# SparkJiao/llama-pipeline-parallel

Hardware: AMD Instinct MI355X
Metric: tokens/sec (whole node), LLaMA-65B PP=8 seq4096 at 1/2/4/8 MI355X (higher is better)
Workload: dtype bf16; 1 GPU; model=llama-65b, measured_model=llama-65b-shaped 10-layer slice (10/80 layers), global_batch=64, seq_len=4096, parallelism=pp1, num_layers=10, micro_batch_size=4, grad_accum_steps=16

## Files before the change

### lpp_amd/ops/csrc/attention_api.cpp

```cpp
#include <string>
#include <vector>

#include "attention.h"

namespace lpp {

static int g_order_mode = [] {
  const char* e = getenv("LPP_ATTN_ORDER");
  return (e && e[0] == '0') ? 0 : 1;
}();

int attn_order_mode() { return g_order_mode; }

void attn_check_qkv(const at::Tensor& q, const at::Tensor& k, const at::Tensor& v,
                    const char* who) {
  TORCH_CHECK(q.is_cuda() && q.scalar_type() == at::kBFloat16, who, ": bf16 only");
  TORCH_CHECK(q.dim() == 4 && q.size(3) == ATTN_D, who, ": [B,S,H,128] required");
  TORCH_CHECK(q.is_contiguous() && k.is_contiguous() && v.is_contiguous());
  TORCH_CHECK(q.size(2) % k.size(2) == 0);
}

static void attn_check_bwd(const at::Tensor& dO, const at::Tensor& q, const at::Tensor& k,
                           const at::Tensor& v, const at::Tensor& o,
                           const at::Tensor& lse2, const char* who) {
// ... 24 lines not shown
  auto dv = at::empty_like(v);
  const int mode = lpp::attn_order_mode();
  lpp::launch_attn_bwd_dq(dO, q, k, v, lse2, delta, dq, mode ? lpp::ATTN_MODE1_DQ : 0, 0);
  lpp::launch_attn_bwd_dkdv(dO, q, k, v, lse2, delta, dk, dv,
                            mode ? lpp::ATTN_MODE1_DKDV : 0, 0);
  return {dq, dk, dv};
}

void attention_set_block_order(int64_t mode) {
  TORCH_CHECK(mode == 0 || mode == 1, "attention_set_block_order: mode 0 or 1");
  lpp::g_order_mode = (int)mode;
}

int64_t attention_get_block_order() { return lpp::g_order_mode; }

at::Tensor attention_block_order(int64_t kind, int64_t nblk, int64_t nheads, int64_t G,
                                 int64_t mode) {
  TORCH_CHECK(kind == 0 || kind == 1, "attention_block_order: kind 0 (fwd/dQ) or 1 (dK/dV)");
  TORCH_CHECK(mode == 0 || mode == 1, "attention_block_order: mode 0 or 1");
  TORCH_CHECK(nblk >= 1 && nheads >= 1 && nblk * nheads < (int64_t)1 << 30 && G >= 1);
  G = std::min(G, nheads);
  const int n = (int)(nblk * nheads);
  auto out = at::empty({n, 2}, at::TensorOptions().dtype(at::kInt));
  int* p = out.data_ptr<int>();
  for (int L = 0; L < n; ++L) {
    const lpp::AttnBlock ob =
        lpp::attn_block_order(L, (int)nblk, (int)nheads, (int)G, (int)kind, (int)mode);
    p[2 * L] = ob.blk;
    p[2 * L + 1] = ob.head;
  }
  return out;
}

std::vector<double> attention_time_kernel(std::string kernel, at::Tensor dO, at::Tensor q,
                                          at::Tensor k, at::Tensor v, at::Tensor o,
                                          at::Tensor lse2, int64_t mode, int64_t G,
                                          int64_t warmup, int64_t reps) {
  lpp::attn_check_bwd(dO, q, k, v, o, lse2, "attention_time_kernel");
  TORCH_CHECK(mode == 0 || mode == 1, "attention_time_kernel: mode 0 or 1");
  TORCH_CHECK(kernel == "fwd" || kernel == "dq" || kernel == "dkdv",
              "attention_time_kernel: kernel is fwd, dq or dkdv");
  const int B = q.size(0), S = q.size(1), H = q.size(2);
  auto delta = at::empty({B, H, S}, q.options().dtype(at::kFloat));
  lpp::launch_attn_bwd_delta(dO, o, delta);
  auto o2 = at::empty_like(q), dq = at::empty_like(q);
  auto lse_out = at::empty_like(lse2);
  auto dk = at::empty_like(k), dv = at::empty_like(v);
  auto launch = [&] {
    if (kernel == "fwd") lpp::launch_attn_fwd(q, k, v, o2, lse_out, (int)mode, (int)G);
    else if (kernel == "dq")
      lpp::launch_attn_bwd_dq(dO, q, k, v, lse2, delta, dq, (int)mode, (int)G);
    else lpp::launch_attn_bwd_dkdv(dO, q, k, v, lse2, delta, dk, dv, (int)mode, (int)G);
  };
  auto stream = lpp::current_stream();
  hipEvent_t e0, e1;
  LPP_CHECK_HIP(hipEventCreate(&e0));
  LPP_CHECK_HIP(hipEventCreate(&e1));
  for (int64_t i = 0; i < warmup; ++i) launch();
  std::vector<double> ms;
  for (int64_t i = 0; i < reps; ++i) {
    LPP_CHECK_HIP(hipEventRecord(e0, stream));
    launch();
    LPP_CHECK_HIP(hipEventRecord(e1, stream));
    LPP_CHECK_HIP(hipEventSynchronize(e1));
    float t = 0.f;
    LPP_CHECK_HIP(hipEventElapsedTime(&t, e0, e1));
// ... 7 lines not shown
```

### lpp_amd/ops/csrc/attention_bwd.hip

```cpp
#include "attention.h"

namespace lpp {

__global__ __launch_bounds__(256) void attn_bwd_delta_kernel(
    const short* __restrict__ dO, const short* __restrict__ O,
    float* __restrict__ delta, int64_t rows, int S, int H) {
  const int lg = threadIdx.x & 15;
  const int grp = (blockIdx.x * 256 + (int)threadIdx.x) >> 4;
  const int64_t stride = ((int64_t)gridDim.x * 256) >> 4;
  for (int64_t r = grp; r < rows; r += stride) {
    const bf16x8 d8 = *reinterpret_cast<const bf16x8*>(&dO[r * ATTN_D + lg * 8]);
    const bf16x8 o8 = *reinterpret_cast<const bf16x8*>(&O[r * ATTN_D + lg * 8]);
    float acc = 0.f;
#pragma unroll
    for (int j = 0; j < 8; ++j) acc += bf16_to_f32(d8[j]) * bf16_to_f32(o8[j]);
#pragma unroll
    for (int m = 1; m < 16; m <<= 1) acc += __shfl_xor(acc, m);
    if (lg == 0) {
      const int h = (int)(r % H);
      const int64_t bs = r / H;
      const int s = (int)(bs % S);
      const int64_t b = bs / S;
      delta[(b * H + h) * S + s] = acc;
    }
  }
}

constexpr int DQ_QW = 32, DQ_QB = 256, DQ_KVB = ATTN_TILE_ROWS;
enum { DQ_K, DQ_V, DQ_KT, DQ_IMAGES };
constexpr int DQ_LDS_BYTES = attn_lds_bytes(DQ_IMAGES);

__global__ __launch_bounds__(512, 2) void attn_bwd_dq_kernel(
    const short* __restrict__ Q, const short* __restrict__ K,
    const short* __restrict__ V, const short* __restrict__ dO,
    const float* __restrict__ LSE2, const float* __restrict__ Delta,
    short* __restrict__ dQ,
    int B, int S, int H, int HKV, float c, float scale,
    int order_mode, int order_G) {
  extern __shared__ __attribute__((aligned(16))) char smem[];
  auto k_lds = [&](int buf) -> char* { return attn_img(smem, DQ_K, buf); };
  auto v_lds = [&](int buf) -> char* { return attn_img(smem, DQ_V, buf); };
  auto kt_lds = [&](int buf) -> char* { return attn_img(smem, DQ_KT, buf); };

  const int tid = threadIdx.x;
  const int wid = __builtin_amdgcn_readfirstlane(tid >> 6);
  const int lane = tid & 63;
  const int lq = lane & 31;
  const int hi2 = lane >> 5;

  const AttnBlock ob = attn_block_order(blockIdx.x, (S + DQ_QB - 1) / DQ_QB, B * H,
                                        order_G, ATTN_ORDER_FWD_DQ, order_mode);
  const int qblk = ob.blk;
  const int b = ob.head / H;
  const int h = ob.head % H;
  const int hkv = h / (H / HKV);
  const int64_t sHD = (int64_t)H * ATTN_D;
  const int64_t sHkvD = (int64_t)HKV * ATTN_D;
  const int64_t q_base = (((int64_t)b * S) * H + h) * ATTN_D;
  const int64_t kv_base = (((int64_t)b * S) * HKV + hkv) * ATTN_D;
  const int64_t ld_base = ((int64_t)b * H + h) * S;

  const int qw0 = qblk * DQ_QB + wid * DQ_QW;
  const int qrow = qw0 + lq;

  bf16x8 qf[8], dof[8];
  {
    const int64_t rb = q_base + (int64_t)min(qrow, S - 1) * sHD;
#pragma unroll
    for (int dc = 0; dc < 8; ++dc) {
      qf[dc] = *reinterpret_cast<const bf16x8*>(&Q[rb + dc * 16 + hi2 * 8]);
      dof[dc] = *reinterpret_cast<const bf16x8*>(&dO[rb + dc * 16 + hi2 * 8]);
    }
  }
  const float Lq = LSE2[ld_base + min(qrow, S - 1)];
  const float Dq = Delta[ld_base + min(qrow, S - 1)];

  const int st_r = lane >> 4;
  const int st_c = 8 * (lane & 15);
  const int kv_end = min(S, (qblk + 1) * DQ_QB);

  auto ld_tile = [&](int kv0, int pass, bf16x8& kreg, bf16x8& vreg) {
    const int row = min(kv0 + stage_row(wid, pass, st_r), S - 1);
    const int64_t rb = kv_base + (int64_t)row * sHkvD + st_c;
    kreg = *reinterpret_cast<const bf16x8*>(&K[rb]);
    vreg = *reinterpret_cast<const bf16x8*>(&V[rb]);
  };
  auto write_tile = [&](int buf, int pass, bf16x8 kreg, bf16x8 vreg) {
    const int r = stage_row(wid, pass, st_r);
    stage_normal(k_lds(buf), r, st_c, kreg);
    stage_normal(v_lds(buf), r, st_c, vreg);
    stage_transposed(kt_lds(buf), r, st_c, st_r, kreg);
  };

  f32x16 dq_acc[4];
#pragma unroll
  for (int dt = 0; dt < 4; ++dt)
#pragma unroll
    for (int r = 0; r < 16; ++r) dq_acc[dt][r] = 0.f;

  bf16x8 kreg0, kreg1, vreg0, vreg1;
  ld_tile(0, 0, kreg0, vreg0);
  ld_tile(0, 1, kreg1, vreg1);
  write_tile(0, 0, kreg0, vreg0);
  write_tile(0, 1, kreg1, vreg1);
  if (DQ_KVB < kv_end) {
    ld_tile(DQ_KVB, 0, kreg0, vreg0);
    ld_tile(DQ_KVB, 1, kreg1, vreg1);
  }
  __syncthreads();
  for (int kv0 = 0, cur = 0; kv0 < kv_end; kv0 += DQ_KVB, cur ^= 1) {
    if (kv0 + DQ_KVB < kv_end) {
      write_tile(cur ^ 1, 0, kreg0, vreg0);
      write_tile(cur ^ 1, 1, kreg1, vreg1);
      if (kv0 + 2 * DQ_KVB < kv_end) {
        ld_tile(kv0 + 2 * DQ_KVB, 0, kreg0, vreg0);
        ld_tile(kv0 + 2 * DQ_KVB, 1, kreg1, vreg1);
      }
    }
    if (kv0 < qw0 + DQ_QW) {
      const bool need_mask = (kv0 + DQ_KVB > qw0) || (kv0 + DQ_KVB > S);
#pragma unroll
      for (int t2 = 0; t2 < 2; ++t2) {
        f32x16 st, dpt;
#pragma unroll
        for (int r = 0; r < 16; ++r) { st[r] = 0.f; dpt[r] = 0.f; }
        __builtin_amdgcn_s_setprio(1);
#pragma unroll
        for (int dc = 0; dc < 8; ++dc) {
          const bf16x8 ak = *reinterpret_cast<const bf16x8*>(
              k_lds(cur) + rswz(t2 * 32 + lq, dc * 16 + hi2 * 8));
          const bf16x8 av = *reinterpret_cast<const bf16x8*>(
              v_lds(cur) + rswz(t2 * 32 + lq, dc * 16 + hi2 * 8));
          st = __builtin_amdgcn_mfma_f32_32x32x16_bf16(ak, qf[dc], st, 0, 0, 0);
          dpt = __builtin_amdgcn_mfma_f32_32x32x16_bf16(av, dof[dc], dpt, 0, 0, 0);
        }
        __builtin_amdgcn_s_setprio(0);

        float ds[16];
        if (need_mask) {
#pragma unroll
          for (int r = 0; r < 16; ++r) {
            const int kv = kv0 + t2 * 32 + crow32(r, hi2);
            const bool ok = (kv <= qrow) && (kv < S);
            const float e = exp2f(fmaf(st[r], c, -Lq));
            ds[r] = (ok ? e : 0.f) * (dpt[r] - Dq);
          }
        } else {
#pragma unroll
          for (int r = 0; r < 16; ++r)
            ds[r] = exp2f(fmaf(st[r], c, -Lq)) * (dpt[r] - Dq);
        }

        bf16x8 dsa[2];
        pack_pair(ds, dsa);

        __builtin_amdgcn_s_setprio(1);
#pragma unroll
        for (int dt = 0; dt < 4; ++dt) {
          const int d = dt * 32 + lq;
#pragma unroll
          for (int ks = 0; ks < 2; ++ks) {
            const bf16x8 bk = *reinterpret_cast<const bf16x8*>(
                kt_lds(cur) + tswz(d, (2 * t2 + ks) * 16 + hi2 * 8));
            dq_acc[dt] = __builtin_amdgcn_mfma_f32_32x32x16_bf16(dsa[ks], bk, dq_acc[dt], 0, 0, 0);
          }
        }
        __builtin_amdgcn_s_setprio(0);
      }
    }
    __syncthreads();
  }

#pragma unroll
  for (int r = 0; r < 16; ++r) {
    const int row = qw0 + crow32(r, hi2);
    if (row >= S) continue;
    const int64_t rb = q_base + (int64_t)row * sHD;
#pragma unroll
    for (int dt = 0; dt < 4; ++dt)
      dQ[rb + dt * 32 + lq] = f32_to_bf16(dq_acc[dt][r] * scale);
  }
}

constexpr int KV_KW = 16, KV_WG = 128, KV_QT = ATTN_TILE_ROWS;
enum { KV_Q, KV_DO, KV_QTR, KV_DOTR, KV_IMAGES };
constexpr int KV_LD_OFF = attn_lds_bytes(KV_IMAGES);
constexpr int KV_D_OFF = KV_LD_OFF + 2 * KV_QT * (int)sizeof(float);
constexpr int KV_LDS_BYTES = KV_D_OFF + 2 * KV_QT * (int)sizeof(float);

__global__ __launch_bounds__(512, 2) void attn_bwd_dkdv_kernel(
    const short* __restrict__ Q, const short* __restrict__ K,
    const short* __restrict__ V, const short* __restrict__ dO,
    const float* __restrict__ LSE2, const float* __restrict__ Delta,
    short* __restrict__ dK, short* __restrict__ dV,
    int B, int S, int H, int HKV, float c, float scale,
    int order_mode, int order_G) {
  extern __shared__ __attribute__((aligned(16))) char smem[];
  auto q_lds = [&](int buf) -> char* { return attn_img(smem, KV_Q, buf); };
  auto do_lds = [&](int buf) -> char* { return attn_img(smem, KV_DO, buf); };
  auto qt_lds = [&](int buf) -> char* { return attn_img(smem, KV_QTR, buf); };
  auto dot_lds = [&](int buf) -> char* { return attn_img(smem, KV_DOTR, buf); };
  auto l_buf = [&](int buf) -> float* {
    return reinterpret_cast<float*>(smem + KV_LD_OFF) + buf * KV_QT; };
  auto d_buf = [&](int buf) -> float* {
    return reinterpret_cast<float*>(smem + KV_D_OFF) + buf * KV_QT; };

  const int tid = threadIdx.x;
  const int wid = __builtin_amdgcn_readfirstlane(tid >> 6);
  const int lane = tid & 63;
  const int l16 = lane & 15;
  const int hi4 = (lane >> 4) & 3;

  const AttnBlock ob = attn_block_order(blockIdx.x, (S + KV_WG - 1) / KV_WG, B * HKV,
                                        order_G, ATTN_ORDER_DKDV, order_mode);
  const int kvblk = ob.blk;
  const int b = ob.head / HKV;
  const int hkv = ob.head % HKV;
  const int G = H / HKV;
  const int64_t sHD = (int64_t)H * ATTN_D;
  const int64_t sHkvD = (int64_t)HKV * ATTN_D;
  const int64_t kv_base = (((int64_t)b * S) * HKV + hkv) * ATTN_D;

  const int kvw0 = kvblk * KV_WG + wid * KV_KW;
  const int kvrow = kvw0 + l16;

  bf16x8 kf[4], vf[4];
  {
    const int64_t rb = kv_base + (int64_t)min(kvrow, S - 1) * sHkvD;
#pragma unroll
    for (int dc = 0; dc < 4; ++dc) {
      kf[dc] = *reinterpret_cast<const bf16x8*>(&K[rb + dc * 32 + hi4 * 8]);
      vf[dc] = *reinterpret_cast<const bf16x8*>(&V[rb + dc * 32 + hi4 * 8]);
    }
  }

  f32x4 dv_acc[8], dk_acc[8];
#pragma unroll
  for (int dt = 0; dt < 8; ++dt)
#pragma unroll
    for (int r = 0; r < 4; ++r) { dv_acc[dt][r] = 0.f; dk_acc[dt][r] = 0.f; }

  const int st_r = (lane >> 4) & 3;
  const int st_c = 8 * (lane & 15);
  const int qstart = kvblk * KV_WG;

  for (int g = 0; g < G; ++g) {
    const int h = hkv * G + g;
    const int64_t q_base = (((int64_t)b * S) * H + h) * ATTN_D;
    const int64_t ld_base = ((int64_t)b * H + h) * S;

    auto ld_tile = [&](int qt0, int pass, bf16x8& qreg, bf16x8& dreg) {
      const int row = min(qt0 + stage_row(wid, pass, st_r), S - 1);
      const int64_t rb = q_base + (int64_t)row * sHD + st_c;
      qreg = *reinterpret_cast<const bf16x8*>(&Q[rb]);
      dreg = *reinterpret_cast<const bf16x8*>(&dO[rb]);
    };
    auto write_tile = [&](int buf, int qt0, int pass, bf16x8 qreg, bf16x8 dreg) {
      const int r = stage_row(wid, pass, st_r);
      stage_normal(q_lds(buf), r, st_c, qreg);
      stage_normal(do_lds(buf), r, st_c, dreg);
      stage_transposed(qt_lds(buf), r, st_c, st_r, qreg);
      stage_transposed(dot_lds(buf), r, st_c, st_r, dreg);
      if (pass == 0 && tid < 128) {
        const int qi = min(qt0 + (tid & 63), S - 1);
        if (tid < 64) l_buf(buf)[tid] = LSE2[ld_base + qi];
        else d_buf(buf)[tid & 63] = Delta[ld_base + qi];
      }
    };

    attn_tile_pipeline<KV_QT>(qstart, S, ld_tile, write_tile, [&](int qt0, int cur) {
      if (qt0 + KV_QT - 1 < kvw0) return;
#pragma unroll
      for (int half = 0; half < 2; ++half) {
        const int qh0 = qt0 + half * 32;
        if (qh0 + 31 < kvw0) continue;
        f32x4 st[2], dpt[2];
#pragma unroll
        for (int qs = 0; qs < 2; ++qs)
#pragma unroll
          for (int r = 0; r < 4; ++r) { st[qs][r] = 0.f; dpt[qs][r] = 0.f; }
        __builtin_amdgcn_s_setprio(1);
#pragma unroll
        for (int dc = 0; dc < 4; ++dc) {
#pragma unroll
          for (int qs = 0; qs < 2; ++qs) {
            const bf16x8 aq = *reinterpret_cast<const bf16x8*>(
                q_lds(cur) + rswz(half * 32 + qs * 16 + l16, dc * 32 + hi4 * 8));
            const bf16x8 ad = *reinterpret_cast<const bf16x8*>(
                do_lds(cur) + rswz(half * 32 + qs * 16 + l16, dc * 32 + hi4 * 8));
            st[qs] = __builtin_amdgcn_mfma_f32_16x16x32_bf16(aq, kf[dc], st[qs], 0, 0, 0);
            dpt[qs] = __builtin_amdgcn_mfma_f32_16x16x32_bf16(ad, vf[dc], dpt[qs], 0, 0, 0);
          }
        }
        __builtin_amdgcn_s_setprio(0);

        const bool need_mask = (qh0 < kvw0 + KV_KW) || (qh0 + 32 > S);
        float p[2][4], ds[2][4];
#pragma unroll
        for (int qs = 0; qs < 2; ++qs) {
          const int q0 = half * 32 + qs * 16 + hi4 * 4;
          const f32x4 Lr = *reinterpret_cast<const f32x4*>(&l_buf(cur)[q0]);
          const f32x4 Dr = *reinterpret_cast<const f32x4*>(&d_buf(cur)[q0]);
          if (need_mask) {
#pragma unroll
            for (int r = 0; r < 4; ++r) {
              const int q = qt0 + q0 + r;
              const bool ok = (kvrow < S) && (q >= kvrow) && (q < S);
              const float e = exp2f(fmaf(st[qs][r], c, -Lr[r]));
              p[qs][r] = ok ? e : 0.f;
              ds[qs][r] = p[qs][r] * (dpt[qs][r] - Dr[r]);
            }
          } else {
#pragma unroll
            for (int r = 0; r < 4; ++r) {
              p[qs][r] = exp2f(fmaf(st[qs][r], c, -Lr[r]));
              ds[qs][r] = p[qs][r] * (dpt[qs][r] - Dr[r]);
            }
          }
        }

        const bf16x8 pa = pack_frag16(p, hi4 & 1);
        const bf16x8 dsa = pack_frag16(ds, hi4 & 1);

        __builtin_amdgcn_s_setprio(1);
#pragma unroll
        for (int dt = 0; dt < 8; ++dt) {
          const int d = dt * 16 + l16;
          const bf16x8 bd = *reinterpret_cast<const bf16x8*>(
              dot_lds(cur) + tswz(d, half * 32 + hi4 * 8));
          const bf16x8 bq = *reinterpret_cast<const bf16x8*>(
              qt_lds(cur) + tswz(d, half * 32 + hi4 * 8));
          dv_acc[dt] = __builtin_amdgcn_mfma_f32_16x16x32_bf16(pa, bd, dv_acc[dt], 0, 0, 0);
          dk_acc[dt] = __builtin_amdgcn_mfma_f32_16x16x32_bf16(dsa, bq, dk_acc[dt], 0, 0, 0);
        }
        __builtin_amdgcn_s_setprio(0);
      }
    });
    __syncthreads();
  }

#pragma unroll
  for (int r = 0; r < 4; ++r) {
    const int row = kvw0 + hi4 * 4 + r;
    if (row >= S) continue;
    const int64_t rb = kv_base + (int64_t)row * sHkvD;
#pragma unroll
    for (int dt = 0; dt < 8; ++dt) {
      dV[rb + dt * 16 + l16] = f32_to_bf16(dv_acc[dt][r]);
      dK[rb + dt * 16 + l16] = f32_to_bf16(dk_acc[dt][r] * scale);
    }
  }
}

void launch_attn_bwd_delta(const at::Tensor& dO, const at::Tensor& o, at::Tensor& delta) {
  const int B = dO.size(0), S = dO.size(1), H = dO.size(2);
  const int64_t rows = (int64_t)B * S * H;
  const int grid = grid_for(rows * 16, 256);
  hipLaunchKernelGGL(attn_bwd_delta_kernel, dim3(grid), dim3(256), 0, current_stream(),
                     (const short*)dO.data_ptr(), (const short*)o.data_ptr(),
                     delta.data_ptr<float>(), rows, S, H);
  LPP_CHECK_HIP(hipGetLastError());
}

void launch_attn_bwd_dq(const at::Tensor& dO, const at::Tensor& q, const at::Tensor& k,
// ... 40 lines not shown
```

### lpp_amd/ops/csrc/attention_fwd.hip

```cpp
#include "attention.h"

namespace lpp {

constexpr int AF_QW = 32;
constexpr int AF_QB = 256;
constexpr int AF_KVB = ATTN_TILE_ROWS;
constexpr float AF_THR = 8.0f;
enum { AF_K, AF_VT, AF_IMAGES };
constexpr int AF_LDS_BYTES = attn_lds_bytes(AF_IMAGES);

__global__ __launch_bounds__(512, 2) void attn_fwd_kernel(
    const short* __restrict__ Q, const short* __restrict__ K,
    const short* __restrict__ V, short* __restrict__ O, float* __restrict__ LSE2,
    int B, int S, int H, int HKV, float c ,
    int order_mode, int order_G) {
  extern __shared__ __attribute__((aligned(16))) char smem[];
  auto k_lds = [&](int buf) -> char* { return attn_img(smem, AF_K, buf); };
  auto vt_lds = [&](int buf) -> char* { return attn_img(smem, AF_VT, buf); };

  const int tid = threadIdx.x;
  const int wid = tid >> 6;
  const int lane = tid & 63;
  const int lq = lane & 31;
  const int hi2 = lane >> 5;

  const AttnBlock ob = attn_block_order(blockIdx.x, (S + AF_QB - 1) / AF_QB, B * H,
                                        order_G, ATTN_ORDER_FWD_DQ, order_mode);
  const int qblk = ob.blk;
  const int bh = ob.head;
  const int b = bh / H;
  const int h = bh % H;
  const int hkv = h / (H / HKV);

  const int64_t sHD = (int64_t)H * ATTN_D;
  const int64_t sHkvD = (int64_t)HKV * ATTN_D;
  const int64_t q_base = (((int64_t)b * S) * H + h) * ATTN_D;
  const int64_t kv_base = (((int64_t)b * S) * HKV + hkv) * ATTN_D;

  const int qw0 = qblk * AF_QB + wid * AF_QW;
  const int qrow = qw0 + lq;

  bf16x8 qf[8];
  {
    const int64_t rb = q_base + (int64_t)min(qrow, S - 1) * sHD;
#pragma unroll
    for (int dc = 0; dc < 8; ++dc)
      qf[dc] = *reinterpret_cast<const bf16x8*>(&Q[rb + dc * 16 + hi2 * 8]);
  }

  const int st_r = (lane >> 4);
  const int st_c = 8 * (lane & 15);

  const int kv_end = min(S, (qblk + 1) * AF_QB);

  auto ld_tile = [&](int kv0, int pass, bf16x8& kreg, bf16x8& vreg) {
    const int row = min(kv0 + stage_row(wid, pass, st_r), S - 1);
    const int64_t rb = kv_base + (int64_t)row * sHkvD + st_c;
    kreg = *reinterpret_cast<const bf16x8*>(&K[rb]);
    vreg = *reinterpret_cast<const bf16x8*>(&V[rb]);
  };
  auto write_tile = [&](int buf, int , int pass, bf16x8 kreg, bf16x8 vreg) {
    const int r = stage_row(wid, pass, st_r);
    stage_normal(k_lds(buf), r, st_c, kreg);
    stage_transposed(vt_lds(buf), r, st_c, st_r, vreg);
  };

  f32x16 o_acc[4];
#pragma unroll
  for (int dt = 0; dt < 4; ++dt)
#pragma unroll
    for (int r = 0; r < 16; ++r) o_acc[dt][r] = 0.f;
  float m_run = -INFINITY, l_run = 0.f;

  attn_tile_pipeline<AF_KVB>(0, kv_end, ld_tile, write_tile, [&](int kv0, int cur) {
    if (kv0 >= qw0 + AF_QW) return;
    f32x16 st[2];
#pragma unroll
    for (int t2 = 0; t2 < 2; ++t2)
#pragma unroll
      for (int r = 0; r < 16; ++r) st[t2][r] = 0.f;
    __builtin_amdgcn_s_setprio(1);
#pragma unroll
    for (int dc = 0; dc < 8; ++dc) {
#pragma unroll
      for (int t2 = 0; t2 < 2; ++t2) {
        const bf16x8 kf = *reinterpret_cast<const bf16x8*>(
            k_lds(cur) + rswz(t2 * 32 + lq, dc * 16 + hi2 * 8));
        st[t2] = __builtin_amdgcn_mfma_f32_32x32x16_bf16(kf, qf[dc], st[t2], 0, 0, 0);
      }
    }
    __builtin_amdgcn_s_setprio(0);

    float ms[32];
    const bool need_mask = (kv0 + AF_KVB > qw0) || (kv0 + AF_KVB > S);
#pragma unroll
    for (int t2 = 0; t2 < 2; ++t2)
#pragma unroll
      for (int r = 0; r < 16; ++r) {
        float v = st[t2][r];
        if (need_mask) {
          const int kv = kv0 + t2 * 32 + crow32(r, hi2);
          if (kv > qrow || kv >= S) v = -INFINITY;
        }
        ms[t2 * 16 + r] = v;
      }

    float pmax = ms[0];
#pragma unroll
    for (int i = 1; i < 32; ++i) pmax = fmaxf(pmax, ms[i]);
    {
      int2v sw = __builtin_amdgcn_permlane32_swap(as_i(pmax), as_i(pmax), false, false);
      pmax = fmaxf(pmax, as_f(hi2 ? sw[0] : sw[1]));
    }
    const float rm2 = pmax * c;

    float m_new = m_run;
    if (__any(rm2 > m_run + AF_THR)) {
      m_new = fmaxf(m_run, rm2);
      const float alpha = (m_run == -INFINITY) ? 0.f : exp2f(m_run - m_new);
      l_run *= alpha;
#pragma unroll
      for (int r = 0; r < 16; ++r) {
        const float ar =
            as_f(__builtin_amdgcn_ds_bpermute(crow32(r, hi2) * 4, as_i(alpha)));
#pragma unroll
        for (int dt = 0; dt < 4; ++dt) o_acc[dt][r] *= ar;
      }
      m_run = m_new;
    }

    float p[32];
    float ps = 0.f;
#pragma unroll
    for (int i = 0; i < 32; ++i) {
      p[i] = exp2f(fmaf(ms[i], c, -m_new));
      ps += p[i];
    }
    {
      int2v sw = __builtin_amdgcn_permlane32_swap(as_i(ps), as_i(ps), false, false);
      ps += as_f(hi2 ? sw[0] : sw[1]);
    }
    l_run += ps;

    bf16x8 pa[4];
    pack_pair(&p[0], &pa[0]);
    pack_pair(&p[16], &pa[2]);

    __builtin_amdgcn_s_setprio(1);
#pragma unroll
    for (int dt = 0; dt < 4; ++dt) {
      const int d = dt * 32 + lq;
#pragma unroll
      for (int ks = 0; ks < 4; ++ks) {
        const bf16x8 bv = *reinterpret_cast<const bf16x8*>(
            vt_lds(cur) + tswz(d, ks * 16 + hi2 * 8));
        o_acc[dt] = __builtin_amdgcn_mfma_f32_32x32x16_bf16(pa[ks], bv, o_acc[dt], 0, 0, 0);
      }
    }
    __builtin_amdgcn_s_setprio(0);
  });

  const float invl = (l_run > 0.f) ? 1.f / l_run : 0.f;
#pragma unroll
  for (int r = 0; r < 16; ++r) {
    const int rq = crow32(r, hi2);
    const float ir = as_f(__builtin_amdgcn_ds_bpermute(rq * 4, as_i(invl)));
    const int row = qw0 + rq;
    if (row >= S) continue;
    const int64_t rb = q_base + (int64_t)row * sHD;
#pragma unroll
    for (int dt = 0; dt < 4; ++dt) O[rb + dt * 32 + lq] = f32_to_bf16(o_acc[dt][r] * ir);
  }
  if (hi2 == 0 && qrow < S)
    LSE2[((int64_t)b * H + h) * S + qrow] = m_run + log2f(l_run);
}

void launch_attn_fwd(const at::Tensor& q, const at::Tensor& k, const at::Tensor& v,
                     at::Tensor& o, at::Tensor& lse2, int order_mode, int order_G) {
  const int B = q.size(0), S = q.size(1), H = q.size(2);
  const int HKV = k.size(2);
  const int qblocks = (S + AF_QB - 1) / AF_QB;
  if (order_G <= 0)
    order_G = attn_order_group(ATTN_GROUP_WAVES * ATTN_RESIDENT_PER_XCD, qblocks);
  hipLaunchKernelGGL(attn_fwd_kernel, dim3(qblocks * B * H), dim3(512), AF_LDS_BYTES,
                     current_stream(), (const short*)q.data_ptr(),
                     (const short*)k.data_ptr(), (const short*)v.data_ptr(),
                     (short*)o.data_ptr(), lse2.data_ptr<float>(), B, S, H, HKV,
                     attn_scale().c, order_mode, order_G);
// ... 5 lines not shown
```

### lpp_amd/ops/csrc/attn_tile.h

```cpp
#pragma once

#include "common.h"

namespace lpp {

typedef __attribute__((ext_vector_type(8))) short bf16x8;
typedef __attribute__((ext_vector_type(16))) float f32x16;
typedef __attribute__((ext_vector_type(4))) float f32x4;
typedef __attribute__((ext_vector_type(2))) int int2v;

constexpr int ATTN_D = 128;
constexpr int ATTN_TILE_ROWS = 64;
constexpr int ATTN_IMG_BYTES = ATTN_TILE_ROWS * ATTN_D * 2;

__device__ __forceinline__ char* attn_img(char* smem, int slot, int buf) {
  return smem + (2 * slot + buf) * ATTN_IMG_BYTES;
}
constexpr int attn_lds_bytes(int images) { return 2 * images * ATTN_IMG_BYTES; }

__device__ __forceinline__ unsigned cvt_pk_bf16(float lo, float hi) {
  unsigned r;
  asm("v_cvt_pk_bf16_f32 %0, %1, %2" : "=v"(r) : "v"(lo), "v"(hi));
  return r;
}
__device__ __forceinline__ float bf16_to_f32(short s) {
  union { unsigned u; float f; } cv;
  cv.u = ((unsigned)(unsigned short)s) << 16;
  return cv.f;
}
__device__ __forceinline__ short f32_to_bf16(float f) {
  __hip_bfloat16 h = __float2bfloat16(f);
  return *reinterpret_cast<short*>(&h);
}
__device__ __forceinline__ float as_f(int v) { return __int_as_float(v); }
__device__ __forceinline__ int as_i(float v) { return __float_as_int(v); }

__device__ __forceinline__ int crow32(int r, int hi2) {
  return (r & 3) + 8 * (r >> 2) + 4 * hi2;
}

__device__ __forceinline__ int rswz(int row, int col_elem) {
  return row * 256 + ((col_elem * 2) ^ ((row & 15) << 4));
}
__device__ __forceinline__ int tswz(int d, int r) {
  return (d * 64 + (r ^ ((((d >> 3) ^ d) & 7) << 3))) * 2;
}

__device__ __forceinline__ void quad_transpose(const bf16x8& v, int p, int out[4]) {
#pragma unroll
  for (int k = 0; k < 4; ++k) out[k] = reinterpret_cast<const int*>(&v)[k];
  {
    int t0 = __shfl_xor(out[(p & 1) ^ 1], 16);
    int t1 = __shfl_xor(out[((p & 1) ^ 1) | 2], 16);
    if (p & 1) { out[0] = t0; out[2] = t1; } else { out[1] = t0; out[3] = t1; }
  }
  {
    int lo = (p & 2) ? 0 : 2;
    int t0 = __shfl_xor(out[lo], 32);
    int t1 = __shfl_xor(out[lo + 1], 32);
    out[lo] = t0; out[lo + 1] = t1;
  }
}

__device__ __forceinline__ void write_transposed(char* img, int r0, int d0,
                                                 const int dw[4]) {
#pragma unroll
  for (int e = 0; e < 2; ++e) {
    const int d = d0 + e;
    unsigned w01 = e ? (((unsigned)dw[0] >> 16) | ((unsigned)dw[1] & 0xffff0000u))
                     : (((unsigned)dw[0] & 0xffffu) | ((unsigned)dw[1] << 16));
    unsigned w23 = e ? (((unsigned)dw[2] >> 16) | ((unsigned)dw[3] & 0xffff0000u))
                     : (((unsigned)dw[2] & 0xffffu) | ((unsigned)dw[3] << 16));
    int2v pair = {(int)w01, (int)w23};
    *reinterpret_cast<int2v*>(img + tswz(d, r0)) = pair;
  }
}

__device__ __forceinline__ int stage_row(int wid, int pass, int p) {
  return 4 * wid + 32 * pass + p;
}
__device__ __forceinline__ void stage_normal(char* img, int r, int c, const bf16x8& v) {
  *reinterpret_cast<bf16x8*>(img + rswz(r, c)) = v;
}
__device__ __forceinline__ void stage_transposed(char* img, int r, int c, int p,
                                                 const bf16x8& v) {
  int dw[4];
  quad_transpose(v, p, dw);
  write_transposed(img, r - p, c + 2 * p, dw);
}

__device__ __forceinline__ void pack_pair(const float p[16], bf16x8 out[2]) {
#pragma unroll
  for (int ksl = 0; ksl < 2; ++ksl) {
    const float* pr = &p[8 * ksl];
    const unsigned x1 = cvt_pk_bf16(pr[0], pr[1]);
    const unsigned x2 = cvt_pk_bf16(pr[2], pr[3]);
    const unsigned y1 = cvt_pk_bf16(pr[4], pr[5]);
    const unsigned y2 = cvt_pk_bf16(pr[6], pr[7]);
    const int2v a = __builtin_amdgcn_permlane32_swap((int)x1, (int)y1, false, false);
    const int2v b = __builtin_amdgcn_permlane32_swap((int)x2, (int)y2, false, false);
    int w[4] = {a[0], b[0], a[1], b[1]};
    out[ksl] = *reinterpret_cast<const bf16x8*>(w);
  }
}

__device__ __forceinline__ bf16x8 pack_frag16(const float p[2][4], int hi4_odd) {
  unsigned X0 = cvt_pk_bf16(p[0][0], p[0][1]);
  unsigned Y0 = cvt_pk_bf16(p[0][2], p[0][3]);
  unsigned X1 = cvt_pk_bf16(p[1][0], p[1][1]);
  unsigned Y1 = cvt_pk_bf16(p[1][2], p[1][3]);
  const int2v ax = __builtin_amdgcn_permlane32_swap((int)X0, (int)X1, false, false);
  const int2v cx = __builtin_amdgcn_permlane16_swap(ax[0], ax[0], false, false);
  const int2v cpx = __builtin_amdgcn_permlane16_swap(ax[1], ax[1], false, false);
  const int2v ay = __builtin_amdgcn_permlane32_swap((int)Y0, (int)Y1, false, false);
  const int2v cy = __builtin_amdgcn_permlane16_swap(ay[0], ay[0], false, false);
  const int2v cpy = __builtin_amdgcn_permlane16_swap(ay[1], ay[1], false, false);
  int w[4];
  w[0] = hi4_odd ? cpx[0] : ax[0];
  w[1] = hi4_odd ? cpy[0] : ay[0];
  w[2] = hi4_odd ? ax[1] : cx[1];
  w[3] = hi4_odd ? ay[1] : cy[1];
// ... 32 lines not shown
```

### lpp_amd/ops/csrc/bindings.cpp

```cpp
#include <torch/extension.h>

#include <string>
#include <tuple>
#include <vector>

std::vector<at::Tensor> rmsnorm_fwd(at::Tensor x, at::Tensor weight, double eps);
std::vector<at::Tensor> rmsnorm_bwd(at::Tensor dy, at::Tensor x, at::Tensor weight,
                                    at::Tensor invrms);
at::Tensor rope_fwd(at::Tensor x, at::Tensor cos_t, at::Tensor sin_t, int64_t pos_offset);
at::Tensor rope_bwd(at::Tensor dy, at::Tensor cos_t, at::Tensor sin_t, int64_t pos_offset);
at::Tensor swiglu_fwd(at::Tensor gate, at::Tensor up);
std::vector<at::Tensor> swiglu_bwd(at::Tensor dy, at::Tensor gate, at::Tensor up);
std::vector<at::Tensor> cross_entropy_fwd(at::Tensor logits, at::Tensor labels);
at::Tensor cross_entropy_bwd(at::Tensor logits, at::Tensor labels, at::Tensor lse,
                             double scale);
std::vector<at::Tensor> attention_fwd(at::Tensor q, at::Tensor k, at::Tensor v);
std::vector<at::Tensor> attention_bwd(at::Tensor dO, at::Tensor q, at::Tensor k,
                                      at::Tensor v, at::Tensor o, at::Tensor lse2);
void attention_set_block_order(int64_t mode);
int64_t attention_get_block_order();
at::Tensor attention_block_order(int64_t kind, int64_t nblk, int64_t nheads, int64_t G,
                                 int64_t mode);
std::vector<double> attention_time_kernel(std::string kernel, at::Tensor dO, at::Tensor q,
                                          at::Tensor k, at::Tensor v, at::Tensor o,
                                          at::Tensor lse2, int64_t mode, int64_t G,
                                          int64_t warmup, int64_t reps);
at::Tensor attention_decode(at::Tensor q, at::Tensor k_new, at::Tensor v_new,
                            at::Tensor k_cache, at::Tensor v_cache, at::Tensor cos_t,
                            at::Tensor sin_t, c10::optional<at::Tensor> positions,
                            c10::optional<at::Tensor> rows,
                            c10::optional<at::Tensor> lengths, int64_t uniform_pos,
                            int64_t max_len, int64_t chunk);
int64_t attention_decode_chunk();
at::Tensor mfma_test_16x16x32(at::Tensor A, at::Tensor B);
void wgrad_f32_accum(at::Tensor x, at::Tensor dy, at::Tensor dw);
void wgrad_f32_accum_pre(at::Tensor xT, at::Tensor dyT, at::Tensor dw);
void wgrad_bf16d_pre(at::Tensor xT, at::Tensor dyT, at::Tensor out);
at::Tensor transpose2d(at::Tensor in);
void accum_bf16_f32(at::Tensor dst, at::Tensor src);
std::vector<std::tuple<int64_t, double, std::string>> wgrad_tune(int64_t T, int64_t in,
                                                                 int64_t out,
                                                                 int64_t reps,
                                                                 int64_t kind);
void wgrad_set_algo(int64_t T, int64_t in, int64_t out, int64_t index, int64_t kind);
std::tuple<int64_t, std::string> wgrad_current_algo(int64_t T, int64_t in, int64_t out,
                                                    int64_t kind);
at::Tensor mfma_test_32x32x16(at::Tensor A, at::Tensor B);
std::vector<at::Tensor> attn_tile_test_roundtrip(at::Tensor tile);
at::Tensor attn_tile_test_pack_pair(at::Tensor x);
at::Tensor attn_tile_test_pack_frag16(at::Tensor x);
void fused_adamw(std::vector<at::Tensor> params, std::vector<at::Tensor> masters,
                 std::vector<at::Tensor> grads, std::vector<at::Tensor> exp_avg,
                 std::vector<at::Tensor> exp_avg_sq, double lr, double beta1, double beta2,
                 double eps, double weight_decay, double bias1, double bias2,
                 double grad_scale);

PYBIND11_MODULE(TORCH_EXTENSION_NAME, m) {
  m.doc() = "lpp_amd gfx950 (MI355X/CDNA4) kernels";
  m.def("rmsnorm_fwd", &rmsnorm_fwd, "RMSNorm forward (y, invrms)");
  m.def("rmsnorm_bwd", &rmsnorm_bwd, "RMSNorm backward (dx, dw)");
  m.def("rope_fwd", &rope_fwd, "RoPE forward");
  m.def("rope_bwd", &rope_bwd, "RoPE backward");
  m.def("swiglu_fwd", &swiglu_fwd, "SwiGLU forward");
  m.def("swiglu_bwd", &swiglu_bwd, "SwiGLU backward (dgate, dup)");
  m.def("cross_entropy_fwd", &cross_entropy_fwd, "fused CE forward (loss_sum, lse, count)");
  m.def("cross_entropy_bwd", &cross_entropy_bwd, "fused CE backward (dlogits)");
  m.def("fused_adamw", &fused_adamw, "fused mixed-precision AdamW");
  m.def("attention_fwd", &attention_fwd, "flash causal attention forward (O, LSE2)");
  m.def("attention_bwd", &attention_bwd, "flash causal attention backward (dQ, dK, dV)");
  m.def("attention_set_block_order", &attention_set_block_order,
        "attention block order: 0 = legacy, 1 = XCD-balanced heavy-first (default, "
        "LPP_ATTN_ORDER)", py::arg("mode"));
  m.def("attention_get_block_order", &attention_get_block_order, "current order mode");
  m.def("attention_block_order", &attention_block_order,
        "host: [n,2] int (blk, head) of linear block ids 0..n-1; kind 0 fwd/dQ, 1 dK/dV",
        py::arg("kind"), py::arg("nblk"), py::arg("nheads"), py::arg("G"), py::arg("mode"));
  m.def("attention_time_kernel", &attention_time_kernel,
        "hipEvent ms per launch of one attention kernel (fwd|dq|dkdv) under an explicit "
        "block order", py::arg("kernel"), py::arg("dO"), py::arg("q"), py::arg("k"),
        py::arg("v"), py::arg("o"), py::arg("lse2"), py::arg("mode"), py::arg("G") = 0,
        py::arg("warmup") = 3, py::arg("reps") = 20);
  m.def("attention_decode", &attention_decode,
        "fused single-token decode: RoPE + KV-cache write + GQA attention over keys 0..p of "
        "each row's cache row -> o [N,1,H,128]; chunk 0 = the compiled-in chunk size",
        py::arg("q"), py::arg("k_new"), py::arg("v_new"), py::arg("k_cache"),
        py::arg("v_cache"), py::arg("cos"), py::arg("sin"), py::arg("positions"),
        py::arg("rows"), py::arg("lengths"), py::arg("uniform_pos"), py::arg("max_len"),
        py::arg("chunk") = 0);
  m.def("attention_decode_chunk", &attention_decode_chunk,
        "keys per workgroup of attention_decode");
  m.def("wgrad_f32_accum", &wgrad_f32_accum, "dW_f32 += dY^T @ X (hipBLASLt, beta=1)");
  m.def("wgrad_f32_accum_pre", &wgrad_f32_accum_pre,
        "dW_f32 += dyT @ xT^T, pre-transposed k-contiguous operands (hipBLASLt, beta=1)");
  m.def("transpose2d", &transpose2d, "bf16/fp16 [R,C] -> [C,R] LDS-tiled transpose");
  m.def("wgrad_bf16d_pre", &wgrad_bf16d_pre,
        "bf16-D pre-transposed wgrad GEMM into a reusable scratch (beta 0)");
  m.def("accum_bf16_f32", &accum_bf16_f32, "dst_f32 += src_bf16 (vectorised)");
  m.def("wgrad_tune", &wgrad_tune,
        "exhaustive hipBLASLt solution sweep for a wgrad shape -> [(index, ms, name)]",
        py::arg("T"), py::arg("in_dim"), py::arg("out"), py::arg("reps"), py::arg("kind") = 0);
  m.def("wgrad_set_algo", &wgrad_set_algo, "pin a hipBLASLt solution index for a shape",
        py::arg("T"), py::arg("in_dim"), py::arg("out"), py::arg("index"), py::arg("kind") = 0);
  m.def("wgrad_current_algo", &wgrad_current_algo,
        "current (heuristic-picked) solution for a shape -> (index, name)",
        py::arg("T"), py::arg("in_dim"), py::arg("out"), py::arg("kind") = 0);
  m.def("mfma_test_16x16x32", &mfma_test_16x16x32, "MFMA layout validation");
  m.def("mfma_test_32x32x16", &mfma_test_32x32x16, "MFMA 32x32x16 layout validation");
  m.def("attn_tile_test_roundtrip", &attn_tile_test_roundtrip,
        "attn_tile.h staging: int16 [64,128] -> (normal, transposed) LDS images read back");
  m.def("attn_tile_test_pack_pair", &attn_tile_test_pack_pair,
        "attn_tile.h pack_pair: fp32 [32,32] in C layout -> int32 [64,2,4] A-fragment words");
  m.def("attn_tile_test_pack_frag16", &attn_tile_test_pack_frag16,
        "attn_tile.h pack_frag16: fp32 [32,16] in C layout -> int32 [64,4] A-fragment words");
}
```

Measured before the change: 23470 tokens/s.

## Use one LDS image per tile with ds_read_tr transposed reads in attention

Drops the separate transposed LDS images for K/V (fwd, dQ) and Q/dO (dK/dV). Each tile is now staged once in a new swizzled layout, and the transposed MFMA B-fragments are read with ds_read_tr16_b64 instead of being built by shuffle-based quad transposes at staging time. This cuts LDS writes, cross-lane shuffles and LDS footprint per stage, which may allow more occupancy or buffering. The risks are bank conflicts from the new swizzle and the latency of the transposed-read instructions. Host helpers and test bindings are added to check the address patterns.

```diff
diff --git a/lpp_amd/ops/csrc/attention_api.cpp b/lpp_amd/ops/csrc/attention_api.cpp
--- a/lpp_amd/ops/csrc/attention_api.cpp
+++ b/lpp_amd/ops/csrc/attention_api.cpp
@@ -80,6 +80,28 @@
   return out;
 }
 
+at::Tensor attention_lds_addresses(std::string pattern, int64_t shape, int64_t idx) {
+  TORCH_CHECK(shape == 32 || shape == 16, "attention_lds_addresses: shape 32 or 16");
+  const bool stage = pattern == "stage", row = pattern == "row", tr = pattern == "tr";
+  TORCH_CHECK(stage || row || tr, "attention_lds_addresses: pattern is stage, row or tr");
+  TORCH_CHECK(idx >= 0 && idx < (tr ? 32 : 16), "attention_lds_addresses: idx out of range");
+  auto out = at::empty({64}, at::TensorOptions().dtype(at::kInt));
+  int* p = out.data_ptr<int>();
+  const int i = (int)idx;
+  for (int lane = 0; lane < 64; ++lane) {
+    if (stage)
+      p[lane] = shape == 32 ? lpp::attn_stage_off<32>(i >> 1, i & 1, lane)
+                            : lpp::attn_stage_off<16>(i >> 1, i & 1, lane);
+    else if (row)
+      p[lane] = shape == 32 ? lpp::attn_row_off32(lane, i >> 3, i & 7)
+                            : lpp::attn_row_off16(lane, i >> 2, i & 3);
+    else
+      p[lane] = shape == 32 ? lpp::attn_tr_off32(lane, i >> 3, (i >> 1) & 3, i & 1)
+                            : lpp::attn_tr_off16(lane, i >> 2, (i >> 1) & 1, i & 1);
+  }
+  return out;
+}
+
 std::vector<double> attention_time_kernel(std::string kernel, at::Tensor dO, at::Tensor q,
                                           at::Tensor k, at::Tensor v, at::Tensor o,
                                           at::Tensor lse2, int64_t mode, int64_t G,
diff --git a/lpp_amd/ops/csrc/attention_bwd.hip b/lpp_amd/ops/csrc/attention_bwd.hip
--- a/lpp_amd/ops/csrc/attention_bwd.hip
+++ b/lpp_amd/ops/csrc/attention_bwd.hip
@@ -27,7 +27,7 @@
 }
 
 constexpr int DQ_QW = 32, DQ_QB = 256, DQ_KVB = ATTN_TILE_ROWS;
-enum { DQ_K, DQ_V, DQ_KT, DQ_IMAGES };
+enum { DQ_K, DQ_V, DQ_IMAGES };
 constexpr int DQ_LDS_BYTES = attn_lds_bytes(DQ_IMAGES);
 
 __global__ __launch_bounds__(512, 2) void attn_bwd_dq_kernel(
@@ -40,7 +40,6 @@
   extern __shared__ __attribute__((aligned(16))) char smem[];
   auto k_lds = [&](int buf) -> char* { return attn_img(smem, DQ_K, buf); };
   auto v_lds = [&](int buf) -> char* { return attn_img(smem, DQ_V, buf); };
-  auto kt_lds = [&](int buf) -> char* { return attn_img(smem, DQ_KT, buf); };
 
   const int tid = threadIdx.x;
   const int wid = __builtin_amdgcn_readfirstlane(tid >> 6);
@@ -77,6 +76,7 @@
 
   const int st_r = lane >> 4;
   const int st_c = 8 * (lane & 15);
+  const int st_off[2] = {attn_stage_off<32>(wid, 0, lane), attn_stage_off<32>(wid, 1, lane)};
   const int kv_end = min(S, (qblk + 1) * DQ_QB);
 
   auto ld_tile = [&](int kv0, int pass, bf16x8& kreg, bf16x8& vreg) {
@@ -86,10 +86,8 @@
     vreg = *reinterpret_cast<const bf16x8*>(&V[rb]);
   };
   auto write_tile = [&](int buf, int pass, bf16x8 kreg, bf16x8 vreg) {
-    const int r = stage_row(wid, pass, st_r);
-    stage_normal(k_lds(buf), r, st_c, kreg);
-    stage_normal(v_lds(buf), r, st_c, vreg);
-    stage_transposed(kt_lds(buf), r, st_c, st_r, kreg);
+    stage_chunk(k_lds(buf), st_off[pass], kreg);
+    stage_chunk(v_lds(buf), st_off[pass], vreg);
   };
 
   f32x16 dq_acc[4];
@@ -127,10 +125,8 @@
         __builtin_amdgcn_s_setprio(1);
 #pragma unroll
         for (int dc = 0; dc < 8; ++dc) {
-          const bf16x8 ak = *reinterpret_cast<const bf16x8*>(
-              k_lds(cur) + rswz(t2 * 32 + lq, dc * 16 + hi2 * 8));
-          const bf16x8 av = *reinterpret_cast<const bf16x8*>(
-              v_lds(cur) + rswz(t2 * 32 + lq, dc * 16 + hi2 * 8));
+          const bf16x8 ak = read_row_frag(k_lds(cur), attn_row_off32(lane, t2, dc));
+          const bf16x8 av = read_row_frag(v_lds(cur), attn_row_off32(lane, t2, dc));
           st = __builtin_amdgcn_mfma_f32_32x32x16_bf16(ak, qf[dc], st, 0, 0, 0);
           dpt = __builtin_amdgcn_mfma_f32_32x32x16_bf16(av, dof[dc], dpt, 0, 0, 0);
         }
@@ -157,11 +153,11 @@
         __builtin_amdgcn_s_setprio(1);
 #pragma unroll
         for (int dt = 0; dt < 4; ++dt) {
-          const int d = dt * 32 + lq;
 #pragma unroll
           for (int ks = 0; ks < 2; ++ks) {
-            const bf16x8 bk = *reinterpret_cast<const bf16x8*>(
-                kt_lds(cur) + tswz(d, (2 * t2 + ks) * 16 + hi2 * 8));
+            const bf16x8 bk =
+                read_tr_frag(k_lds(cur), attn_tr_off32(lane, dt, 2 * t2 + ks, 0),
+                             attn_tr_off32(lane, dt, 2 * t2 + ks, 1));
             dq_acc[dt] = __builtin_amdgcn_mfma_f32_32x32x16_bf16(dsa[ks], bk, dq_acc[dt], 0, 0, 0);
           }
         }
@@ -183,7 +179,7 @@
 }
 
 constexpr int KV_KW = 16, KV_WG = 128, KV_QT = ATTN_TILE_ROWS;
-enum { KV_Q, KV_DO, KV_QTR, KV_DOTR, KV_IMAGES };
+enum { KV_Q, KV_DO, KV_IMAGES };
 constexpr int KV_LD_OFF = attn_lds_bytes(KV_IMAGES);
 constexpr int KV_D_OFF = KV_LD_OFF + 2 * KV_QT * (int)sizeof(float);
 constexpr int KV_LDS_BYTES = KV_D_OFF + 2 * KV_QT * (int)sizeof(float);
@@ -198,8 +194,6 @@
   extern __shared__ __attribute__((aligned(16))) char smem[];
   auto q_lds = [&](int buf) -> char* { return attn_img(smem, KV_Q, buf); };
   auto do_lds = [&](int buf) -> char* { return attn_img(smem, KV_DO, buf); };
-  auto qt_lds = [&](int buf) -> char* { return attn_img(smem, KV_QTR, buf); };
-  auto dot_lds = [&](int buf) -> char* { return attn_img(smem, KV_DOTR, buf); };
   auto l_buf = [&](int buf) -> float* {
     return reinterpret_cast<float*>(smem + KV_LD_OFF) + buf * KV_QT; };
   auto d_buf = [&](int buf) -> float* {
@@ -242,6 +236,7 @@
 
   const int st_r = (lane >> 4) & 3;
   const int st_c = 8 * (lane & 15);
+  const int st_off[2] = {attn_stage_off<16>(wid, 0, lane), attn_stage_off<16>(wid, 1, lane)};
   const int qstart = kvblk * KV_WG;
 
   for (int g = 0; g < G; ++g) {
@@ -256,11 +251,8 @@
       dreg = *reinterpret_cast<const bf16x8*>(&dO[rb]);
     };
     auto write_tile = [&](int buf, int qt0, int pass, bf16x8 qreg, bf16x8 dreg) {
-      const int r = stage_row(wid, pass, st_r);
-      stage_normal(q_lds(buf), r, st_c, qreg);
-      stage_normal(do_lds(buf), r, st_c, dreg);
-      stage_transposed(qt_lds(buf), r, st_c, st_r, qreg);
-      stage_transposed(dot_lds(buf), r, st_c, st_r, dreg);
+      stage_chunk(q_lds(buf), st_off[pass], qreg);
+      stage_chunk(do_lds(buf), st_off[pass], dreg);
       if (pass == 0 && tid < 128) {
         const int qi = min(qt0 + (tid & 63), S - 1);
         if (tid < 64) l_buf(buf)[tid] = LSE2[ld_base + qi];
@@ -284,10 +276,9 @@
         for (int dc = 0; dc < 4; ++dc) {
 #pragma unroll
           for (int qs = 0; qs < 2; ++qs) {
-            const bf16x8 aq = *reinterpret_cast<const bf16x8*>(
-                q_lds(cur) + rswz(half * 32 + qs * 16 + l16, dc * 32 + hi4 * 8));
-            const bf16x8 ad = *reinterpret_cast<const bf16x8*>(
-                do_lds(cur) + rswz(half * 32 + qs * 16 + l16, dc * 32 + hi4 * 8));
+            const int off = attn_row_off16(lane, 2 * half + qs, dc);
+            const bf16x8 aq = read_row_frag(q_lds(cur), off);
+            const bf16x8 ad = read_row_frag(do_lds(cur), off);
             st[qs] = __builtin_amdgcn_mfma_f32_16x16x32_bf16(aq, kf[dc], st[qs], 0, 0, 0);
             dpt[qs] = __builtin_amdgcn_mfma_f32_16x16x32_bf16(ad, vf[dc], dpt[qs], 0, 0, 0);
           }
@@ -325,11 +316,10 @@
         __builtin_amdgcn_s_setprio(1);
 #pragma unroll
         for (int dt = 0; dt < 8; ++dt) {
-          const int d = dt * 16 + l16;
-          const bf16x8 bd = *reinterpret_cast<const bf16x8*>(
-              dot_lds(cur) + tswz(d, half * 32 + hi4 * 8));
-          const bf16x8 bq = *reinterpret_cast<const bf16x8*>(
-              qt_lds(cur) + tswz(d, half * 32 + hi4 * 8));
+          const int off0 = attn_tr_off16(lane, dt, half, 0);
+          const int off1 = attn_tr_off16(lane, dt, half, 1);
+          const bf16x8 bd = read_tr_frag(do_lds(cur), off0, off1);
+          const bf16x8 bq = read_tr_frag(q_lds(cur), off0, off1);
           dv_acc[dt] = __builtin_amdgcn_mfma_f32_16x16x32_bf16(pa, bd, dv_acc[dt], 0, 0, 0);
           dk_acc[dt] = __builtin_amdgcn_mfma_f32_16x16x32_bf16(dsa, bq, dk_acc[dt], 0, 0, 0);
         }
diff --git a/lpp_amd/ops/csrc/attention_fwd.hip b/lpp_amd/ops/csrc/attention_fwd.hip
--- a/lpp_amd/ops/csrc/attention_fwd.hip
+++ b/lpp_amd/ops/csrc/attention_fwd.hip
@@ -6,7 +6,7 @@
 constexpr int AF_QB = 256;
 constexpr int AF_KVB = ATTN_TILE_ROWS;
 constexpr float AF_THR = 8.0f;
-enum { AF_K, AF_VT, AF_IMAGES };
+enum { AF_K, AF_V, AF_IMAGES };
 constexpr int AF_LDS_BYTES = attn_lds_bytes(AF_IMAGES);
 
 __global__ __launch_bounds__(512, 2) void attn_fwd_kernel(
@@ -16,10 +16,10 @@
     int order_mode, int order_G) {
   extern __shared__ __attribute__((aligned(16))) char smem[];
   auto k_lds = [&](int buf) -> char* { return attn_img(smem, AF_K, buf); };
-  auto vt_lds = [&](int buf) -> char* { return attn_img(smem, AF_VT, buf); };
+  auto v_lds = [&](int buf) -> char* { return attn_img(smem, AF_V, buf); };
 
   const int tid = threadIdx.x;
-  const int wid = tid >> 6;
+  const int wid = __builtin_amdgcn_readfirstlane(tid >> 6);
   const int lane = tid & 63;
   const int lq = lane & 31;
   const int hi2 = lane >> 5;
@@ -50,6 +50,7 @@
 
   const int st_r = (lane >> 4);
   const int st_c = 8 * (lane & 15);
+  const int st_off[2] = {attn_stage_off<32>(wid, 0, lane), attn_stage_off<32>(wid, 1, lane)};
 
   const int kv_end = min(S, (qblk + 1) * AF_QB);
 
@@ -60,9 +61,8 @@
     vreg = *reinterpret_cast<const bf16x8*>(&V[rb]);
   };
   auto write_tile = [&](int buf, int , int pass, bf16x8 kreg, bf16x8 vreg) {
-    const int r = stage_row(wid, pass, st_r);
-    stage_normal(k_lds(buf), r, st_c, kreg);
-    stage_transposed(vt_lds(buf), r, st_c, st_r, vreg);
+    stage_chunk(k_lds(buf), st_off[pass], kreg);
+    stage_chunk(v_lds(buf), st_off[pass], vreg);
   };
 
   f32x16 o_acc[4];
@@ -84,8 +84,7 @@
     for (int dc = 0; dc < 8; ++dc) {
 #pragma unroll
       for (int t2 = 0; t2 < 2; ++t2) {
-        const bf16x8 kf = *reinterpret_cast<const bf16x8*>(
-            k_lds(cur) + rswz(t2 * 32 + lq, dc * 16 + hi2 * 8));
+        const bf16x8 kf = read_row_frag(k_lds(cur), attn_row_off32(lane, t2, dc));
         st[t2] = __builtin_amdgcn_mfma_f32_32x32x16_bf16(kf, qf[dc], st[t2], 0, 0, 0);
       }
     }
@@ -149,11 +148,10 @@
     __builtin_amdgcn_s_setprio(1);
 #pragma unroll
     for (int dt = 0; dt < 4; ++dt) {
-      const int d = dt * 32 + lq;
 #pragma unroll
       for (int ks = 0; ks < 4; ++ks) {
-        const bf16x8 bv = *reinterpret_cast<const bf16x8*>(
-            vt_lds(cur) + tswz(d, ks * 16 + hi2 * 8));
+        const bf16x8 bv = read_tr_frag(v_lds(cur), attn_tr_off32(lane, dt, ks, 0),
+                                       attn_tr_off32(lane, dt, ks, 1));
         o_acc[dt] = __builtin_amdgcn_mfma_f32_32x32x16_bf16(pa[ks], bv, o_acc[dt], 0, 0, 0);
       }
     }
diff --git a/lpp_amd/ops/csrc/attn_tile.h b/lpp_amd/ops/csrc/attn_tile.h
--- a/lpp_amd/ops/csrc/attn_tile.h
+++ b/lpp_amd/ops/csrc/attn_tile.h
@@ -5,6 +5,7 @@
 namespace lpp {
 
 typedef __attribute__((ext_vector_type(8))) short bf16x8;
+typedef __attribute__((ext_vector_type(4))) short bf16x4;
 typedef __attribute__((ext_vector_type(16))) float f32x16;
 typedef __attribute__((ext_vector_type(4))) float f32x4;
 typedef __attribute__((ext_vector_type(2))) int int2v;
@@ -39,54 +40,71 @@
   return (r & 3) + 8 * (r >> 2) + 4 * hi2;
 }
 
-__device__ __forceinline__ int rswz(int row, int col_elem) {
-  return row * 256 + ((col_elem * 2) ^ ((row & 15) << 4));
+#define ATTN_HD __host__ __device__ __forceinline__
+
+ATTN_HD int attn_swz32(int row) { return ((row & 3) << 2) | ((row >> 2) & 3); }
+ATTN_HD int attn_swz16(int row) {
+  const int a = row & 3, b = (row >> 2) & 3;
+  return (a << 1) | (((b ^ (b >> 1)) & 1) << 3) | (b >> 1);
 }
-__device__ __forceinline__ int tswz(int d, int r) {
-  return (d * 64 + (r ^ ((((d >> 3) ^ d) & 7) << 3))) * 2;
+template <int M>
+ATTN_HD int attn_off(int row, int ch) {
+  static_assert(M == 32 || M == 16, "MFMA shape: 32 (32x32x16) or 16 (16x16x32)");
+  return 256 * row + 16 * (ch ^ (M == 32 ? attn_swz32(row) : attn_swz16(row)));
 }
 
-__device__ __forceinline__ void quad_transpose(const bf16x8& v, int p, int out[4]) {
-#pragma unroll
-  for (int k = 0; k < 4; ++k) out[k] = reinterpret_cast<const int*>(&v)[k];
-  {
-    int t0 = __shfl_xor(out[(p & 1) ^ 1], 16);
-    int t1 = __shfl_xor(out[((p & 1) ^ 1) | 2], 16);
-    if (p & 1) { out[0] = t0; out[2] = t1; } else { out[1] = t0; out[3] = t1; }
-  }
-  {
-    int lo = (p & 2) ? 0 : 2;
-    int t0 = __shfl_xor(out[lo], 32);
-    int t1 = __shfl_xor(out[lo + 1], 32);
-    out[lo] = t0; out[lo + 1] = t1;
-  }
+ATTN_HD int stage_row(int wid, int pass, int p) { return 4 * wid + 32 * pass + p; }
+template <int M>
+ATTN_HD int attn_stage_off(int wid, int pass, int lane) {
+  return attn_off<M>(stage_row(wid, pass, lane >> 4), lane & 15);
 }
 
-__device__ __forceinline__ void write_transposed(char* img, int r0, int d0,
-                                                 const int dw[4]) {
-#pragma unroll
-  for (int e = 0; e < 2; ++e) {
-    const int d = d0 + e;
-    unsigned w01 = e ? (((unsigned)dw[0] >> 16) | ((unsigned)dw[1] & 0xffff0000u))
-                     : (((unsigned)dw[0] & 0xffffu) | ((unsigned)dw[1] << 16));
-    unsigned w23 = e ? (((unsigned)dw[2] >> 16) | ((unsigned)dw[3] & 0xffff0000u))
-                     : (((unsigned)dw[2] & 0xffffu) | ((unsigned)dw[3] << 16));
-    int2v pair = {(int)w01, (int)w23};
-    *reinterpret_cast<int2v*>(img + tswz(d, r0)) = pair;
-  }
+ATTN_HD int attn_row_base32(int lane) { return attn_off<32>(lane & 31, lane >> 5); }
+ATTN_HD int attn_row_at32(int base, int t2, int dc) {
+  return (base ^ (32 * dc)) + 32 * 256 * t2;
+}
+ATTN_HD int attn_row_off32(int lane, int t2, int dc) {
+  return attn_row_at32(attn_row_base32(lane), t2, dc);
+}
+ATTN_HD int attn_row_base16(int lane) { return attn_off<16>(lane & 15, lane >> 4); }
+ATTN_HD int attn_row_at16(int base, int rt, int dc) {
+  return (base ^ (64 * dc)) + 16 * 256 * rt;
+}
+ATTN_HD int attn_row_off16(int lane, int rt, int dc) {
+  return attn_row_at16(attn_row_base16(lane), rt, dc);
+}
+ATTN_HD int attn_tr_base32(int lane) {
+  const int q = (lane >> 2) & 3, p = lane & 3;
+  return attn_off<32>((lane >> 5) * 8 + q, 2 * ((lane >> 4) & 1) + (p >> 1)) + 8 * (p & 1);
+}
+ATTN_HD int attn_tr_at32(int base, int dt, int ks, int h) {
+  return (base ^ (64 * dt + 16 * h)) + 4 * 256 * h + 16 * 256 * ks;
+}
+ATTN_HD int attn_tr_off32(int lane, int dt, int ks, int h) {
+  return attn_tr_at32(attn_tr_base32(lane), dt, ks, h);
+}
+ATTN_HD int attn_tr_base16(int lane) {
+  const int q = (lane >> 2) & 3, p = lane & 3;
+  return attn_off<16>((lane >> 4) * 8 + q, p >> 1) + 8 * (p & 1);
+}
+ATTN_HD int attn_tr_at16(int base, int dt, int half, int h) {
+  return (base ^ (32 * dt) ^ (128 * h)) + 4 * 256 * h + 32 * 256 * half;
+}
+ATTN_HD int attn_tr_off16(int lane, int dt, int half, int h) {
+  return attn_tr_at16(attn_tr_base16(lane), dt, half, h);
 }
 
-__device__ __forceinline__ int stage_row(int wid, int pass, int p) {
-  return 4 * wid + 32 * pass + p;
+__device__ __forceinline__ void stage_chunk(char* img, int off, const bf16x8& v) {
+  *reinterpret_cast<bf16x8*>(img + off) = v;
 }
-__device__ __forceinline__ void stage_normal(char* img, int r, int c, const bf16x8& v) {
-  *reinterpret_cast<bf16x8*>(img + rswz(r, c)) = v;
+__device__ __forceinline__ bf16x8 read_row_frag(const char* img, int off) {
+  return *reinterpret_cast<const bf16x8*>(img + off);
 }
-__device__ __forceinline__ void stage_transposed(char* img, int r, int c, int p,
-                                                 const bf16x8& v) {
-  int dw[4];
-  quad_transpose(v, p, dw);
-  write_transposed(img, r - p, c + 2 * p, dw);
+__device__ __forceinline__ bf16x8 read_tr_frag(const char* img, int off0, int off1) {
+  typedef __attribute__((address_space(3))) bf16x4 lds_bf16x4;
+  const bf16x4 lo = __builtin_amdgcn_ds_read_tr16_b64_v4i16((lds_bf16x4*)(img + off0));
+  const bf16x4 hi = __builtin_amdgcn_ds_read_tr16_b64_v4i16((lds_bf16x4*)(img + off1));
+  return __builtin_shufflevector(lo, hi, 0, 1, 2, 3, 4, 5, 6, 7);
 }
 
 __device__ __forceinline__ void pack_pair(const float p[16], bf16x8 out[2]) {
diff --git a/lpp_amd/ops/csrc/bindings.cpp b/lpp_amd/ops/csrc/bindings.cpp
--- a/lpp_amd/ops/csrc/bindings.cpp
+++ b/lpp_amd/ops/csrc/bindings.cpp
@@ -21,6 +21,7 @@
 int64_t attention_get_block_order();
 at::Tensor attention_block_order(int64_t kind, int64_t nblk, int64_t nheads, int64_t G,
                                  int64_t mode);
+at::Tensor attention_lds_addresses(std::string pattern, int64_t shape, int64_t idx);
 std::vector<double> attention_time_kernel(std::string kernel, at::Tensor dO, at::Tensor q,
                                           at::Tensor k, at::Tensor v, at::Tensor o,
                                           at::Tensor lse2, int64_t mode, int64_t G,
@@ -47,6 +48,8 @@
                                                     int64_t kind);
 at::Tensor mfma_test_32x32x16(at::Tensor A, at::Tensor B);
 std::vector<at::Tensor> attn_tile_test_roundtrip(at::Tensor tile);
+at::Tensor attn_tile_test_tr_fragments(at::Tensor tile, int64_t shape, int64_t nrows,
+                                       int64_t buf);
 at::Tensor attn_tile_test_pack_pair(at::Tensor x);
 at::Tensor attn_tile_test_pack_frag16(at::Tensor x);
 void fused_adamw(std::vector<at::Tensor> params, std::vector<at::Tensor> masters,
@@ -107,7 +110,15 @@
   m.def("mfma_test_16x16x32", &mfma_test_16x16x32, "MFMA layout validation");
   m.def("mfma_test_32x32x16", &mfma_test_32x32x16, "MFMA 32x32x16 layout validation");
   m.def("attn_tile_test_roundtrip", &attn_tile_test_roundtrip,
-        "attn_tile.h staging: int16 [64,128] -> (normal, transposed) LDS images read back");
+        "attn_tile.h dual-use image: int16 [64,128] -> (tile by row reads, transpose by "
+        "transposed reads) from one LDS image");
+  m.def("attn_tile_test_tr_fragments", &attn_tile_test_tr_fragments,
+        "attn_tile.h transposed reads: int16 [64,128] -> int16 [16,64,8], the B-fragments "
+        "of MFMA shape 32 (frag = dt*4+ks) or 16 (frag = dt*2+half) as the kernels read them",
+        py::arg("tile"), py::arg("shape"), py::arg("nrows") = 64, py::arg("buf") = 0);
+  m.def("attention_lds_addresses", &attention_lds_addresses,
+        "host: int32 [64] per-lane LDS byte addresses of one access pattern (stage | row | "
+        "tr) of MFMA shape 32 or 16", py::arg("pattern"), py::arg("shape"), py::arg("idx"));
   m.def("attn_tile_test_pack_pair", &attn_tile_test_pack_pair,
         "attn_tile.h pack_pair: fp32 [32,32] in C layout -> int32 [64,2,4] A-fragment words");
   m.def("attn_tile_test_pack_frag16", &attn_tile_test_pack_frag16,
```

After: 23870 tokens/s, median of 6. 1.02x the previous value.
